# sdiehl/sonic

Measured on AMD Instinct MI355X. Metric: prove() proofs/sec, higher is better.
Workload: dtype u32 limbs (Fq 12x32, Fr 8x32 Montgomery); 1 GPU; prove(): rndCircuit n=2^18, Q=2, SRS d=2^21 (d=8n >= 7n, Protocol.hs:54); n=262144, Q=2, d=2097152, process_group=none (plain single-process run), legs=headline only (the other legs: --full)

## Files before the change

### include/sonic_hip.h

```cpp
#ifndef SONIC_HIP_H
#define SONIC_HIP_H
#include <stddef.h>
#include <stdint.h>

#if defined(__GNUC__)
#pragma GCC visibility push(default)
#endif
#ifdef __cplusplus
extern "C" {
#endif

enum {
  SONIC_OK = 0,
  SONIC_ERR_D_TOO_SMALL = 1,
  SONIC_ERR_SRS_INDEX = 2,
  SONIC_ERR_BAD_ENCODING = 3,
  SONIC_ERR_INEXACT_DIVISION = 4,
  SONIC_ERR_HIP = 5,
  SONIC_ERR_NO_DEVICE = 6,
  SONIC_ERR_INVALID_ARG = 7
};

#define SONIC_FR_BYTES 32
#define SONIC_G1_BYTES 96
// ... 47 lines not shown
int sonic_msm_g1_srs(const sonic_srs_t* srs, int basis, int64_t e0, const uint8_t* scalars, int64_t n,
                     uint8_t out_g1[96]);
int sonic_msm_g1_srs_dev(const sonic_srs_t* srs, int basis, int64_t e0, const void* d_scalars, int64_t n,
                         uint8_t out_g1[96]);
int sonic_msm_g1_srs_partial_dev(const sonic_srs_t* srs, int basis, int64_t e0, const void* d_scalars,
                                 int64_t n, uint8_t out_partial[192]);
int sonic_msm_g2(const uint8_t* points , const uint8_t* scalars , int64_t n, uint8_t out_g2[192]);
int sonic_msm_g2_srs(const sonic_srs_t* srs, int basis, int64_t e0, const uint8_t* scalars, int64_t n, uint8_t out_g2[192]);
int sonic_msm_g2_srs_dev(const sonic_srs_t* srs, int basis, int64_t e0, const void* d_scalars, int64_t n, uint8_t out_g2[192]);
int sonic_msm_g2_walk_max(void);
typedef struct sonic_msm_lane sonic_msm_lane_t;
int sonic_msm_lane_new(sonic_msm_lane_t** out);
int sonic_msm_lane_new_on(int device, sonic_msm_lane_t** out);
void sonic_msm_lane_free(sonic_msm_lane_t* lane);
int sonic_msm_submit(sonic_msm_lane_t* lane, const sonic_srs_t* srs, int basis, int64_t e0, const void* d_scalars, int64_t n);
int sonic_msm_collect(sonic_msm_lane_t* lane, uint8_t* out_g1, uint8_t* out_partial);
int sonic_msm_lane_new_on_stream(void* hip_stream, sonic_msm_lane_t** out);
int sonic_msm_submit_dev_v2(sonic_msm_lane_t* lane, const sonic_srs_t* srs, int basis, int64_t e0, const void* d_scalars, int64_t n,
                            void* d_partial_out, size_t out_bytes);
int sonic_msm_submit_dev(sonic_msm_lane_t* lane, const sonic_srs_t* srs, int basis, int64_t e0, const void* d_scalars, int64_t n,
                         void* d_partial_out);
int sonic_msm_exchange_layout(const sonic_srs_t* srs, int world, int64_t* n_buckets, int64_t* slice_len);
int sonic_msm_accumulate_dev(sonic_msm_lane_t* lane, const sonic_srs_t* srs, int basis, int64_t e0, const void* d_scalars, int64_t n,
                             void* d_buckets, int64_t capacity);
int sonic_msm_reduce_slices_dev_v2(sonic_msm_lane_t* lane, const sonic_srs_t* srs, const void* d_slices, int k, int64_t slice_len,
                                   int64_t bucket_base, void* d_partial_out, size_t out_bytes);
int sonic_msm_reduce_slices_dev(sonic_msm_lane_t* lane, const sonic_srs_t* srs, const void* d_slices, int k, int64_t slice_len,
                                int64_t bucket_base, void* d_partial_out);
int sonic_msm_lane_sync(sonic_msm_lane_t* lane);
int sonic_g1_sum_partials(const uint8_t* partials, int k, uint8_t out_g1[96]);
int sonic_g1_sum_dev_partials(const uint8_t* blobs, int k, uint8_t out_g1[96]);
int sonic_ntt_fr(uint8_t* data, int log2n, int inverse);
int sonic_poly_mul_fr(const uint8_t* a, int64_t na, const uint8_t* b, int64_t nb, uint8_t* out);
int sonic_poly_mul_fr_dev(const void* d_a, int64_t na, const void* d_b, int64_t nb, void* d_out);
int sonic_srs_point_bytes(void);
int sonic_msm_set_window(int c);
int sonic_msm_plan(const sonic_srs_t* srs, int64_t n, int* window_bits, int* windows, int* bucket_sets);

size_t sonic_proof_size(int64_t Q);
int sonic_prove(const sonic_srs_t* srs, int64_t n, int64_t Q, const uint8_t* wL, const uint8_t* wR,
                const uint8_t* wO, const uint8_t* cs, const uint8_t* aL, const uint8_t* aR,
                const uint8_t* aO, const uint8_t* transcript, uint8_t* out_proof);
int sonic_one_shot_trim(int device);
int sonic_prover_new(const sonic_srs_t* srs, int64_t n, int64_t Q, const uint8_t* wL, const uint8_t* wR,
                     const uint8_t* wO, const uint8_t* cs, sonic_prover_t** out);
int sonic_prover_new_csr(const sonic_srs_t* srs, int64_t n, int64_t Q, const int64_t* row_ptr, const int64_t* col, const uint8_t* val,
                         const uint8_t* cs, sonic_prover_t** out);
int sonic_prove_csr(const sonic_srs_t* srs, int64_t n, int64_t Q, const int64_t* row_ptr, const int64_t* col, const uint8_t* val,
                    const uint8_t* cs, const uint8_t* aL, const uint8_t* aR, const uint8_t* aO, const uint8_t* transcript,
                    uint8_t* out_proof);
int sonic_prover_set_assignment(sonic_prover_t* p, const uint8_t* aL, const uint8_t* aR, const uint8_t* aO);
int sonic_prover_prepare(sonic_prover_t* p);
int sonic_prover_prove(sonic_prover_t* p, const uint8_t* transcript, uint8_t* out_proof);
int sonic_prover_submit(sonic_prover_t* p, const uint8_t* transcript);
int sonic_prover_collect(sonic_prover_t* p, uint8_t* out_proof);
void sonic_prover_free(sonic_prover_t* p);

int sonic_prover_set_share(sonic_prover_t* p, int rank, int world);
size_t sonic_proof_share_size(int64_t Q);
int sonic_prover_prove_share(sonic_prover_t* p, const uint8_t* transcript, uint8_t* out_share);
int sonic_prover_collect_share(sonic_prover_t* p, uint8_t* out_share);
int sonic_proof_from_shares(int64_t Q, int world, const uint8_t* shares, const uint8_t* transcript, uint8_t* out_proof);
int sonic_prove_share_plan(int64_t n, int64_t Q, int prepared, int world, int rank, int64_t nb, int w, uint32_t* out_lo_hi, double* out_cost);

typedef struct sonic_statement {
  const uint8_t *wL, *wR, *wO, *cs;
// ... 190 lines not shown
```

### sonic_amd/_lib.py

```python
from __future__ import annotations

import ctypes as C
import os
import sys
import warnings

_HERE = os.path.dirname(os.path.abspath(__file__))
LIB_PATH = os.environ.get("SONIC_HIP_LIB") or os.path.join(_HERE, "csrc", "libsonic_hip.so")

ERR_NAMES = {
    1: "D_TOO_SMALL", 2: "SRS_INDEX_OUT_OF_RANGE", 3: "BAD_ENCODING", 4: "INEXACT_DIVISION",
    5: "HIP_ERROR", 6: "NO_DEVICE", 7: "INVALID_ARG",
}


class SonicError(RuntimeError):
    def __init__(self, code: int, message: str):
        super().__init__(f"{ERR_NAMES.get(code, code)}: {message}")
        self.code = code
        self.message = message


_lib = None

# ... 44 lines not shown
        "sonic_prove_batch": [vp, i32, i64, vp, vp, vp, vp, vp, vp],
        "sonic_prove_many": [vp, i32, i64, i64, vp, i64, vp, vp],
        "sonic_one_shot_trim": [i32],
        "sonic_msm_g1_srs_multi": [vp, i32, i32, i64, vp, i64, i32, vp],
        "sonic_msm_g1_srs_multi_dev": [vp, i32, i32, vp, vp, vp, i32, vp],
        "sonic_prover_device": [vp],
        "sonic_dev_alloc_on": [i32, C.c_size_t, C.POINTER(vp)],
        "sonic_srs_get_points": [vp, i32, i64, i64, vp],
        "sonic_srs_get_g2_points": [vp, i32, i64, i64, vp],
        "sonic_srs_save": [vp, cp, i32],
        "sonic_srs_has_g2": [vp],
        "sonic_srs_set_g2_points": [vp, vp, vp],
        "sonic_srs_load": [cp, C.POINTER(vp)],
        "sonic_commit_poly": [vp, i64, i64, vp, vp, vp],
        "sonic_open_poly": [vp, cp, i64, vp, vp, vp, vp],
        "sonic_msm_g1": [vp, vp, i64, vp],
        "sonic_msm_g1_srs": [vp, i32, i64, vp, i64, vp],
        "sonic_msm_g1_srs_dev": [vp, i32, i64, vp, i64, vp],
        "sonic_msm_g1_srs_partial_dev": [vp, i32, i64, vp, i64, vp],
        "sonic_g1_sum_partials": [vp, i32, vp],
        "sonic_g1_sum_dev_partials": [vp, i32, vp],
        "sonic_msm_lane_new": [C.POINTER(vp)],
        "sonic_msm_submit": [vp, vp, i32, i64, vp, i64],
        "sonic_msm_collect": [vp, vp, vp],
        "sonic_msm_lane_new_on_stream": [vp, C.POINTER(vp)],
        "sonic_msm_submit_dev_v2": [vp, vp, i32, i64, vp, i64, vp, C.c_size_t],
        "sonic_msm_exchange_layout": [vp, i32, C.POINTER(i64), C.POINTER(i64)],
        "sonic_msm_accumulate_dev": [vp, vp, i32, i64, vp, i64, vp, i64],
        "sonic_msm_reduce_slices_dev_v2": [vp, vp, vp, i32, i64, i64, vp, C.c_size_t],
        "sonic_msm_lane_sync": [vp],
        "sonic_ntt_fr": [vp, i32, i32],
        "sonic_poly_mul_fr": [vp, i64, vp, i64, vp],
        "sonic_poly_mul_fr_dev": [vp, i64, vp, i64, vp],
        "sonic_msm_set_window": [i32],
        "sonic_srs_point_bytes": [],
        "sonic_msm_plan": [vp, i64, C.POINTER(i32), C.POINTER(i32), C.POINTER(i32)],
        "sonic_prove": [vp, i64, i64] + [vp] * 9,
        "sonic_prover_new": [vp, i64, i64, vp, vp, vp, vp, C.POINTER(vp)],
        "sonic_prover_new_csr": [vp, i64, i64, vp, vp, vp, vp, C.POINTER(vp)],
        "sonic_prove_csr": [vp, i64, i64] + [vp] * 9,
        "sonic_fs_circuit_digest_csr": [i64, i64, vp, vp, vp, vp, vp],
        "sonic_verify_csr": [vp, i64, i64, vp, vp, vp, vp, vp, cp, cp, vp, C.POINTER(i32)],
        "sonic_verify_fs_csr": [vp, i64, i64, vp, vp, vp, vp, vp, C.POINTER(i32)],
        "sonic_prover_set_assignment": [vp, vp, vp, vp],
        "sonic_prover_prove": [vp, vp, vp],
        "sonic_prover_submit": [vp, vp],
        "sonic_prover_collect": [vp, vp],
        "sonic_prover_prepare": [vp],
        "sonic_prover_set_share": [vp, i32, i32],
        "sonic_prover_prove_share": [vp, vp, vp],
        "sonic_prover_collect_share": [vp, vp],
        "sonic_proof_from_shares": [i64, i32, vp, vp, vp],
        "sonic_prove_share_plan": [i64, i64, i32, i32, i32, i64, i32, vp, C.POINTER(C.c_double)],
        "sonic_fs_circuit_digest": [i64, i64, vp, vp, vp, vp, vp],
        "sonic_prover_prove_fs": [vp, cp, cp, vp, vp],
        "sonic_fs_srs_id": [vp, vp],
        "sonic_fs_challenges_v2": [i64, i64, i64, cp, cp, vp, vp],
        "sonic_verify_fs": [vp, i64, i64, vp, vp, vp, vp, vp, C.POINTER(i32)],
        "sonic_prover_hsc_prove": [vp, i64, vp, cp, cp, vp],
        "sonic_hsc_prove_poly": [vp, i64, vp, vp, vp, i64, vp, cp, cp, vp],
        "sonic_hsc_verify_poly": [vp, i64, vp, vp, vp, i64, vp, vp, C.POINTER(i32)],
        "sonic_hsc_verify": [vp, i64, i64, vp, vp, vp, i64, vp, vp, C.POINTER(i32)],
        "sonic_pc_v": [vp, i64, cp, cp, cp, cp, C.POINTER(i32)],
        "sonic_verify": [vp, i64, i64, vp, vp, vp, vp, vp, cp, cp, vp, C.POINTER(i32)],
        "sonic_verifier_new": [vp, i64, i64, vp, vp, vp, vp, C.POINTER(vp)],
        "sonic_verifier_new_csr": [vp, i64, i64, vp, vp, vp, vp, C.POINTER(vp)],
# ... 140 lines not shown
EXPORTED = [
    "sonic_abi_version", "sonic_device_count", "sonic_srs_new_on", "sonic_srs_from_points_on", "sonic_srs_replicate", "sonic_srs_device", "sonic_srs_pairing",
    "sonic_srs_load_on", "sonic_msm_lane_new_on", "sonic_msm_submit_dev_v2", "sonic_msm_reduce_slices_dev_v2", "sonic_fs_challenges_v2",
    "sonic_prove_shared", "sonic_prove_batch", "sonic_prove_many", "sonic_one_shot_trim", "sonic_msm_g1_srs_multi", "sonic_msm_g1_srs_multi_dev", "sonic_prover_device", "sonic_dev_alloc_on",
    "sonic_init", "sonic_last_error", "sonic_device_sync", "sonic_hip_versions", "sonic_srs_new", "sonic_srs_from_points",
    "sonic_srs_free", "sonic_srs_d", "sonic_srs_get_points", "sonic_srs_get_g2_points", "sonic_srs_set_g2_points", "sonic_srs_save", "sonic_srs_has_g2", "sonic_srs_load", "sonic_commit_poly", "sonic_open_poly",
    "sonic_msm_g1", "sonic_msm_g1_srs", "sonic_msm_g1_srs_dev", "sonic_msm_g1_srs_partial_dev",
    "sonic_g1_sum_partials", "sonic_g1_sum_dev_partials", "sonic_msm_lane_new", "sonic_msm_lane_free", "sonic_msm_submit", "sonic_msm_collect", "sonic_msm_lane_new_on_stream", "sonic_msm_submit_dev", "sonic_msm_exchange_layout",
    "sonic_msm_accumulate_dev", "sonic_msm_reduce_slices_dev", "sonic_msm_lane_sync", "sonic_ntt_fr", "sonic_poly_mul_fr", "sonic_poly_mul_fr_dev", "sonic_msm_set_window", "sonic_srs_point_bytes", "sonic_msm_plan",
    "sonic_proof_size", "sonic_prove", "sonic_prover_new", "sonic_prover_set_assignment",
    "sonic_prover_prove", "sonic_prover_submit", "sonic_prover_collect", "sonic_prover_prepare",
    "sonic_prover_set_share", "sonic_proof_share_size", "sonic_prover_prove_share", "sonic_prover_collect_share", "sonic_proof_from_shares", "sonic_prove_share_plan", "sonic_fs_circuit_digest", "sonic_fs_srs_id", "sonic_prover_prove_fs", "sonic_fs_challenges", "sonic_verify_fs", "sonic_prover_hsc_prove", "sonic_hsc_prove_poly", "sonic_hsc_verify_poly", "sonic_hsc_proof_size", "sonic_hsc_verify", "sonic_prover_free", "sonic_pc_v", "sonic_verify", "sonic_dev_alloc", "sonic_dev_free", "sonic_dev_upload",
    "sonic_dev_download", "sonic_profile_enable", "sonic_profile_reset", "sonic_profile_get",
    "sonic_profile_names",
    "sonic_prover_new_csr", "sonic_prove_csr", "sonic_fs_circuit_digest_csr", "sonic_verify_csr", "sonic_verify_fs_csr",
    "sonic_verifier_new", "sonic_verifier_new_csr", "sonic_verifier_free", "sonic_verifier_device", "sonic_verifier_verify_batch", "sonic_verifier_verify_fs_batch",
    "sonic_verifier_eval_s", "sonic_g1_validate", "sonic_verify_batch_randomizers",
    "sonic_g1_compress", "sonic_g1_decompress", "sonic_g2_compress", "sonic_g2_decompress", "sonic_proof_size_compressed", "sonic_proof_compress", "sonic_proof_decompress",
    "sonic_verifier_verify_batch_z", "sonic_verifier_verify_fs_batch_z", "sonic_srs_save_compressed",
    "sonic_prover_eval_constraints", "sonic_prover_set_constants", "sonic_prove_batch_statements", "sonic_fs_circuit_midstate", "sonic_fs_circuit_midstate_csr",
    "sonic_fs_circuit_digest_resume", "sonic_verifier_verify_batch_cs", "sonic_verifier_verify_fs_batch_cs", "sonic_verify_batch_digest_v2",
    "sonic_prover_witness_digest_v2", "sonic_prover_submit_fs", "sonic_prover_collect_fs", "sonic_prove_batch_fs",
    "sonic_prover_set_witness", "sonic_prover_eval_constraints_src", "sonic_prove_batch_src", "sonic_prove_batch_fs_src",
    "sonic_srs_for_circuit", "sonic_srs_load_for_circuit", "sonic_srs_load_for_circuit_on", "sonic_srs_windows", "sonic_srs_device_bytes",
    "sonic_prover_prove_core", "sonic_prover_submit_core", "sonic_prover_collect_core", "sonic_prover_prove_core_fs", "sonic_fs_core_challenges",
    "sonic_prove_batch_core_src", "sonic_prove_batch_core_fs_src", "sonic_verify_core", "sonic_verify_core_csr", "sonic_verify_core_fs", "sonic_verify_core_fs_csr",
    "sonic_verifier_verify_core_batch", "sonic_verifier_verify_core_fs_batch", "sonic_verify_core_batch_digest", "sonic_core_proof_compress", "sonic_core_proof_decompress",
    "sonic_fs_weights_digest", "sonic_fs_aggregate_challenges", "sonic_prover_aggregate_core", "sonic_verify_core_helped_digest",
    "sonic_verifier_verify_core_batch_helped", "sonic_verifier_verify_core_fs_batch_helped",
    "sonic_srs_check", "sonic_srs_update", "sonic_srs_verify_update",
    "sonic_msm_g2", "sonic_msm_g2_srs", "sonic_msm_g2_srs_dev", "sonic_msm_g2_walk_max",
    "sonic_g1_subgroup_check", "sonic_g2_subgroup_check",
    "sonic_pairing_check",
]


def last_error() -> str:
    buf = C.create_string_buffer(512)
    lib().sonic_last_error(buf, 512)
    return buf.value.decode(errors="replace")


def check(rc: int) -> None:
    if rc != 0:
        raise SonicError(rc, last_error())
```

### sonic_amd/csrc/poly.hip

```cpp
#include "internal.hpp"
#include "poly.hpp"
#include "csr.hpp"

namespace sonic {

#ifndef SONIC_SCALE_PER
#define SONIC_SCALE_PER 32
#endif
constexpr int SCALE_PER = SONIC_SCALE_PER;
static int scale_per(long n) {
  long per = n / (256L * 64L);
  if (per > SCALE_PER) per = SCALE_PER;
  if (per < 2) per = 2;
  return (int)per;
}

template <int MODE>
__global__ __launch_bounds__(256) void k_scale_powers(const Fr* __restrict__ in, Fr* __restrict__ out, long n, long e0,
                                                      const Fr* __restrict__ px, const Fr* __restrict__ pxinv, long lo_q, long nF, int PER) {
  const long base = (long)blockIdx.x * (256 * PER) + threadIdx.x;
  if (base >= n) return;
  const Fr x = *px, xinv = *pxinv;
  const long e = e0 + base;
  Fr p = e >= 0 ? fp_pow_u64(x, (uint64_t)e) : fp_pow_u64(xinv, (uint64_t)(-e));
// ... 59 lines not shown
  __shared__ Fr sh[256];
  __shared__ Fr carry_sh;
  if (threadIdx.x == 0) carry_sh = Fr::zero();
  __syncthreads();
  for (long base = 0; base < ntiles; base += 256) {
    long idx = base + threadIdx.x;
    Fr v = idx < ntiles ? tile_sums[idx] : Fr::zero();
    Fr incl = block_inclusive_scan_fr(v, sh);
    Fr carry = carry_sh;
    if (idx < ntiles) tile_sums[idx] = fp_add(fp_sub(incl, v), carry);
    __syncthreads();
    if (threadIdx.x == 255) carry_sh = fp_add(carry, incl);
    __syncthreads();
  }
}
__global__ __launch_bounds__(256) void k_prefix_apply(Fr* __restrict__ d, long n, const Fr* __restrict__ tile_sums) {
  const long i = (long)blockIdx.x * 256 + threadIdx.x;
  if (i >= n) return;
  const long tile = i >> 10;
  if (tile == 0) return;
  d[i] = fp_add(d[i], tile_sums[tile]);
}
void poly_prefix_sum_enqueue(hipStream_t st, Fr* d, long n, DevBuf& tmp) {
  if (n <= 0) return;
  const long ntiles = (n + 1023) / 1024;
  tmp.ensure(sizeof(Fr) * (ntiles + 1));
  LAUNCH(k_prefix_tiles, (int)ntiles, 256, 0, st, d, n, tmp.as<Fr>());
  if (ntiles > 1) {
    LAUNCH(k_prefix_top, 1, 256, 0, st, tmp.as<Fr>(), ntiles);
    LAUNCH(k_prefix_apply, ceil_div(n, 256), 256, 0, st, d, n, (const Fr*)tmp.as<Fr>());
  }
}

template <int MODE>
__global__ __launch_bounds__(256) void k_scale_powers_b(const OpenBatch b, long n, long e0, long lo_q, long nF, int PER, int tile_log) {
  const int y = blockIdx.y;
  const long base = (long)blockIdx.x * (256 * PER) + threadIdx.x;
  const Fr* __restrict__ in = MODE == 0 ? b.poly[y] : b.D[y];
  const Fr* __restrict__ tiles = b.tiles[y];
  Fr* __restrict__ out = MODE == 0 ? b.D[y] : b.q[y];
  Fr F;
  if (MODE == 2) {
    F = in[nF - 1];
    if (((nF - 1) >> tile_log) > 0) F = fp_add(F, tiles[(nF - 1) >> tile_log]);
    if (blockIdx.x == 0 && threadIdx.x == 0) *b.fz[y] = F;
  }
  if (base >= n) return;
  const Fr x = MODE == 0 ? b.zpair[y][0] : b.zpair[y][1], xinv = MODE == 0 ? b.zpair[y][1] : b.zpair[y][0];
  const long e = e0 + base;
  Fr p = e >= 0 ? fp_pow_u64(x, (uint64_t)e) : fp_pow_u64(xinv, (uint64_t)(-e));
  const Fr step = fp_pow_u64(x, 256);
#pragma unroll 1
  for (int k = 0; k < PER; k++) {
    const long i = base + (long)k * 256;
    if (i >= n) break;
    Fr v;
    if (MODE == 0) v = fp_mul(in[i], p);
    else {
      Fr P = in[i];
      if ((i >> tile_log) > 0) P = fp_add(P, tiles[i >> tile_log]);
      v = fp_mul((lo_q + i >= 0) ? fp_sub(F, P) : fp_neg(P), p);
    }
    out[i] = v;
    p = fp_mul(p, step);
  }
}
template <int EPT>
__global__ __launch_bounds__(256) void k_prefix_tiles_b(const OpenBatch b, long n) {
  __shared__ Fr sh[256];
  Fr* __restrict__ d = b.D[blockIdx.y];
  const long base = (long)blockIdx.x * (256 * EPT) + threadIdx.x * EPT;
  Fr s = Fr::zero();
  for (int k = 0; k < EPT; k++) if (base + k < n) s = fp_add(s, d[base + k]);
  Fr incl = block_inclusive_scan_fr(s, sh);
  Fr run = fp_sub(incl, s);
  for (int k = 0; k < EPT; k++) if (base + k < n) { run = fp_add(run, d[base + k]); d[base + k] = run; }
  if (threadIdx.x == 255) b.tiles[blockIdx.y][blockIdx.x] = incl;
}
__global__ __launch_bounds__(256) void k_prefix_top_b(const OpenBatch b, long ntiles) {
  __shared__ Fr sh[256];
  __shared__ Fr carry_sh;
  Fr* __restrict__ tile_sums = b.tiles[blockIdx.x];
  if (threadIdx.x == 0) carry_sh = Fr::zero();
  __syncthreads();
  for (long base = 0; base < ntiles; base += 256) {
    long idx = base + threadIdx.x;
    Fr v = idx < ntiles ? tile_sums[idx] : Fr::zero();
    Fr incl = block_inclusive_scan_fr(v, sh);
    Fr carry = carry_sh;
    if (idx < ntiles) tile_sums[idx] = fp_add(fp_sub(incl, v), carry);
    __syncthreads();
    if (threadIdx.x == 255) carry_sh = fp_add(carry, incl);
    __syncthreads();
  }
}
__global__ void k_last_prefix_b(const OpenBatch b, long len, int tile_log) {
  const int y = blockIdx.x;
  Fr F = b.D[y][len - 1];
  if (((len - 1) >> tile_log) > 0) F = fp_add(F, b.tiles[y][(len - 1) >> tile_log]);
  *b.fz[y] = F;
}
void open_batch_enqueue(hipStream_t st, const OpenBatch& b, long lo, long len, bool quotient) {
  if (b.k <= 0 || len <= 0) return;
  const unsigned k = (unsigned)b.k;
  const int tile_log = len >= 65536 ? 12 : 10;
  const int per = scale_per(len);
  LAUNCH(k_scale_powers_b<0>, dim3((unsigned)ceil_div(len, 256L * per), k), 256, 0, st, b, len, lo, 0L, 0L, per, tile_log);
  const long ntiles = (len + (1L << tile_log) - 1) >> tile_log;
  if (tile_log == 12) LAUNCH(k_prefix_tiles_b<16>, dim3((unsigned)ntiles, k), 256, 0, st, b, len);
  else LAUNCH(k_prefix_tiles_b<4>, dim3((unsigned)ntiles, k), 256, 0, st, b, len);
  if (ntiles > 1) LAUNCH(k_prefix_top_b, k, 256, 0, st, b, ntiles);
  if (!quotient) { LAUNCH(k_last_prefix_b, k, 1, 0, st, b, len, tile_log); return; }
  const long qn = len > 1 ? len - 1 : 1;
  const int per2 = scale_per(qn);
  LAUNCH(k_scale_powers_b<2>, dim3((unsigned)ceil_div(qn, 256L * per2), k), 256, 0, st, b, len - 1 > 0 ? len - 1 : 0, 1 + lo, lo, len, per2, tile_log);
}

__global__ __launch_bounds__(256) void k_build_r1(const Fr* __restrict__ aL, const Fr* __restrict__ aR, const Fr* __restrict__ aO,
                                                  const Fr* __restrict__ cns, long n, Fr* __restrict__ r1) {
  const long len = 3 * n + 5;
  for (long i = (long)blockIdx.x * 256 + threadIdx.x; i < len; i += (long)gridDim.x * 256) {
    const long e = i - (2 * n + 4);
    Fr v = Fr::zero();
    if (e > 0) v = aL[e - 1];
    else if (e < 0 && e >= -n) v = aR[-e - 1];
    else if (e < -n && e >= -2 * n) v = aO[-e - n - 1];
    else if (e < -2 * n) v = cns[-e - 2 * n - 1];
    r1[i] = v;
  }
}
void build_r1_enqueue(hipStream_t st, const Fr* aL, const Fr* aR, const Fr* aO, const Fr* cns, long n, Fr* r1) {
  LAUNCH(k_build_r1, elementwise_grid(3 * n + 5), 256, 0, st, aL, aR, aO, cns, n, r1);
}

__global__ __launch_bounds__(256) void k_s_of_y(const Fr* __restrict__ wL, const Fr* __restrict__ wR, const Fr* __restrict__ wO,
                                                const Fr* __restrict__ ypow, long n, long Q, Fr* __restrict__ s) {
  for (long i = (long)blockIdx.x * 256 + threadIdx.x + 1; i <= n + 1; i += (long)gridDim.x * 256) {
    if (i > n) { s[n] = Fr::zero(); break; }
    Fr u = Fr::zero(), v = Fr::zero(), w = Fr::zero();
    for (long q = 0; q < Q; q++) {
      const Fr yq = ypow[2 * n + 1 + q];
      u = fp_add(u, fp_mul(wL[q * n + i - 1], yq));
      v = fp_add(v, fp_mul(wR[q * n + i - 1], yq));
      w = fp_add(w, fp_mul(wO[q * n + i - 1], yq));
    }
    w = fp_sub(fp_sub(w, ypow[n + i]), ypow[n - i]);
    s[n - i] = u;
    s[n + i] = v;
// ... 311 lines not shown
```

### sonic_amd/csrc/poly.hpp

```cpp
#pragma once
#include "common.hpp"
#include "field.hpp"
#include "g1.hpp"

namespace sonic {

void build_r1_enqueue(hipStream_t st, const Fr* aL, const Fr* aR, const Fr* aO, const Fr* cns, long n, Fr* r1);
void s_of_y_enqueue(hipStream_t st, const Fr* wL, const Fr* wR, const Fr* wO, const Fr* ypow, long n, long Q, Fr* s);
void weight_row_poly_enqueue(hipStream_t st, const Fr* wL, const Fr* wR, const Fr* wO, long n, long q, Fr* s);
void s_diag_part_enqueue(hipStream_t st, const Fr* ypow, long n, long Q, Fr* diag, Fr* yq);
void s_of_u_enqueue(hipStream_t st, const Fr* wL, const Fr* wR, const Fr* wO, const Fr* upow, long n, long Q, Fr* s, DevBuf& tmp);
void s_of_y_csc_enqueue(hipStream_t st, const int32_t* col_ptr, const int32_t* row, const Fr* val, const Fr* ypow, long n, long Q, Fr* s);
void s_of_u_csr_enqueue(hipStream_t st, const int32_t* row_ptr, const int32_t* col, const Fr* val, const int32_t* chunk_row, const int32_t* chunk_begin,
                        long nchunks, const int32_t* row_chunk, const Fr* upow, long n, long Q, Fr* s, Fr* partial);
void csr_row_terms_enqueue(hipStream_t st, const int32_t* col, const Fr* val, const int32_t seg[6], long n, PointArray A, G1Affine* pts, Fr* scal);
void add_into_enqueue(hipStream_t st, Fr* dst, const Fr* src, long n);
void t_operands_enqueue(hipStream_t st, const Fr* r1, long r_len, long r_lo, const Fr* sy, long s_off, long s_len, const Fr* ypair, Fr* fa, Fr* fb, long M);
void sub_k_of_y_enqueue(hipStream_t st, Fr* slot, const Fr* cs, const Fr* ypow_nq, long Q, int* flags, int flag_bit);
void flag_nonzero_enqueue(hipStream_t st, const Fr* a, long n, int* flags, int bit);
constexpr int RUN_TILE = 256;
void run_tiles_enqueue(hipStream_t st, const Fr* poly, long len, Fr* masked, Fr* val, uint32_t* uniform);
void run_terms_enqueue(hipStream_t st, const Fr* val, const uint32_t* uniform, long ntiles, PointArray ps, long ps_first, Fr* scal, G1Affine* pts);
void fr_with_inverse_enqueue(hipStream_t st, const Fr* in, int k, Fr* out);
void fr_mul_scalar_enqueue(hipStream_t st, const Fr* a, const Fr* b, Fr* out);
void scale_terms_enqueue(hipStream_t st, const int64_t* e, const Fr* c, long nt, const Fr* pair, Fr* out);
void sparse_to_dense_enqueue(hipStream_t st, const int64_t* exps, const Fr* coeffs, long nt, long lo, Fr* dense);

constexpr int OPEN_BATCH_MAX = 16;
struct OpenBatch {
  int k;
  const Fr* poly[OPEN_BATCH_MAX];
  Fr* D[OPEN_BATCH_MAX];
  Fr* q[OPEN_BATCH_MAX];
  Fr* tiles[OPEN_BATCH_MAX];
  const Fr* zpair[OPEN_BATCH_MAX];
  Fr* fz[OPEN_BATCH_MAX];
};
void open_batch_enqueue(hipStream_t st, const OpenBatch& b, long lo, long len, bool quotient = true);

}
```

### sonic_amd/csrc/poly_api.hip

```cpp
#include "prover.hpp"

extern "C" {

struct BivTerms {
  long nt = 0, lo = 0, len = 0;
  DevBuf keep, other, coeff;
};
static int biv_upload(hipStream_t st, int64_t nt, const int64_t* keep, const int64_t* other, const uint8_t* coeffs, BivTerms& out, int* d_flags) {
  out.nt = nt;
  long lo = 0, hi = 0;
  for (int64_t i = 0; i < nt; i++) { lo = std::min<long>(lo, keep[i]); hi = std::max<long>(hi, keep[i]); }
  out.lo = lo; out.len = hi - lo + 1;
  std::vector<int64_t> order(nt), k(nt), o(nt);
  std::iota(order.begin(), order.end(), 0);
  std::stable_sort(order.begin(), order.end(), [&](int64_t a, int64_t b) { return keep[a] < keep[b]; });
  std::vector<uint8_t> c(32 * (size_t)(nt ? nt : 1));
  for (int64_t i = 0; i < nt; i++) { k[i] = keep[order[i]]; o[i] = other[order[i]]; memcpy(&c[32 * (size_t)i], coeffs + 32 * order[i], 32); }
  out.keep.alloc(8 * (size_t)(nt ? nt : 1)); out.other.alloc(8 * (size_t)(nt ? nt : 1)); out.coeff.alloc(32 * (size_t)(nt ? nt : 1));
  if (nt) {
    HIP_OK(hipMemcpyAsync(out.keep.p, k.data(), 8 * (size_t)nt, hipMemcpyHostToDevice, st));
    HIP_OK(hipMemcpyAsync(out.other.p, o.data(), 8 * (size_t)nt, hipMemcpyHostToDevice, st));
    HIP_OK(hipMemcpyAsync(out.coeff.p, c.data(), 32 * (size_t)nt, hipMemcpyHostToDevice, st));
    fr_to_mont_enqueue(st, out.coeff.as<Fr>(), nt, d_flags);
  }
// ... 205 lines not shown
}

int sonic_poly_mul_fr(const uint8_t* a, int64_t na, const uint8_t* b, int64_t nb, uint8_t* out) {
  API_BEGIN
  if (!a || !b || !out || na < 1 || nb < 1) return SONIC_ERR_INVALID_ARG;
  std::lock_guard<std::mutex> g(call_mutex());
  hipStream_t st = default_stream();
  const long rl = na + nb - 1;
  int lg = 0;
  while ((1L << lg) < rl) lg++;
  const long M = 1L << lg;
  DevBuf fa(sizeof(Fr) * M), fb(sizeof(Fr) * M), flags(4);
  HIP_OK(hipMemsetAsync(flags.p, 0, 4, st));
  HIP_OK(hipMemsetAsync(fa.p, 0, sizeof(Fr) * M, st));
  HIP_OK(hipMemsetAsync(fb.p, 0, sizeof(Fr) * M, st));
  HIP_OK(hipMemcpyAsync(fa.p, a, 32 * na, hipMemcpyHostToDevice, st));
  HIP_OK(hipMemcpyAsync(fb.p, b, 32 * nb, hipMemcpyHostToDevice, st));
  fr_to_mont_enqueue(st, fa.as<Fr>(), na, flags.as<int>());
  fr_to_mont_enqueue(st, fb.as<Fr>(), nb, flags.as<int>());
  if (lg > 0) {
    shared_ntt().ensure(st, lg);
    ntt_forward_enqueue(st, shared_ntt(), fa.as<Fr>(), lg);
    ntt_forward_enqueue(st, shared_ntt(), fb.as<Fr>(), lg);
  }
  if (lg > 0) ntt_inverse_of_product_enqueue(st, shared_ntt(), fa.as<Fr>(), fb.as<Fr>(), lg);
  else fr_pointwise_mul_enqueue(st, fa.as<Fr>(), fb.as<Fr>(), M);
  fr_from_mont_enqueue(st, fa.as<Fr>(), rl);
  int fl = read_flags(st, flags);
  if (fl) return flags_to_status(fl, "sonic_poly_mul_fr");
  HIP_OK(hipMemcpy(out, fa.p, 32 * rl, hipMemcpyDeviceToHost));
  API_END
}

int sonic_poly_mul_fr_dev(const void* d_a, int64_t na, const void* d_b, int64_t nb, void* d_out) {
  API_BEGIN
  if (!d_a || !d_b || !d_out || na < 1 || nb < 1) return SONIC_ERR_INVALID_ARG;
  std::lock_guard<std::mutex> g(call_mutex());
  hipStream_t st = default_stream();
  const long rl = na + nb - 1;
  int lg = 0;
  while ((1L << lg) < rl) lg++;
  const long M = 1L << lg;
  DeviceCtx& dctx = current_ctx();
  DevBuf *fa = &dctx.mul_a, *fb = &dctx.mul_b, *flags = &dctx.mul_flags;
  fa->ensure(sizeof(Fr) * M); fb->ensure(sizeof(Fr) * M); flags->ensure(4);
  HIP_OK(hipMemsetAsync(flags->p, 0, 4, st));
  HIP_OK(hipMemsetAsync(fa->p, 0, sizeof(Fr) * M, st));
  HIP_OK(hipMemsetAsync(fb->p, 0, sizeof(Fr) * M, st));
  HIP_OK(hipMemcpyAsync(fa->p, d_a, 32 * na, hipMemcpyDeviceToDevice, st));
  HIP_OK(hipMemcpyAsync(fb->p, d_b, 32 * nb, hipMemcpyDeviceToDevice, st));
  fr_to_mont_enqueue(st, fa->as<Fr>(), na, flags->as<int>());
  fr_to_mont_enqueue(st, fb->as<Fr>(), nb, flags->as<int>());
  if (lg > 0) {
    shared_ntt().ensure(st, lg);
    ntt_forward_enqueue(st, shared_ntt(), fa->as<Fr>(), lg);
    ntt_forward_enqueue(st, shared_ntt(), fb->as<Fr>(), lg);
  }
  if (lg > 0) ntt_inverse_of_product_enqueue(st, shared_ntt(), fa->as<Fr>(), fb->as<Fr>(), lg);
  else fr_pointwise_mul_enqueue(st, fa->as<Fr>(), fb->as<Fr>(), M);
  fr_from_mont_enqueue(st, fa->as<Fr>(), rl);
  HIP_OK(hipMemcpyAsync(d_out, fa->p, 32 * rl, hipMemcpyDeviceToDevice, st));
  int fl = read_flags(st, *flags);
  if (fl) return flags_to_status(fl, "sonic_poly_mul_fr_dev");
  API_END
}

// ... 2 lines not shown
```

### sonic_amd/csrc/prove.hip

```cpp
#include "prover.hpp"
#include "witness_tree.hpp"

namespace sonic {

constexpr long PROVE_TWO_LEVEL_MAX_TERMS = 1L << 21;
constexpr long POOL_MAX_TERMS = 1L << 21;
static bool prove_two_level(const MsmPlan& pl, int k, bool last, long nmax) {
  if (last || k <= 1 || pl.NB < (1 << 18)) return false;
  const char* e = getenv("SONIC_PROVE_TWO_LEVEL");
  if (e && (e[0] == '0' || e[0] == '1') && !e[1]) return e[0] == '1';
  return nmax <= PROVE_TWO_LEVEL_MAX_TERMS;
}
static int prove_segment(const MsmPlan& pl, int k, bool last, bool two_level) {
  const bool big = pl.NB >= (1 << 18);
  if (last) return big ? 16 : 4;
  if (k <= 1) return big ? 8 : 4;
  if (!big) return 16;
  const char* e = getenv("SONIC_PROVE_SEGMENT");
  const int v = e ? atoi(e) : 0;
  return v >= 8 && v <= 1024 ? v : (two_level ? 32 : 64);
}

MsmJob commit_job(hipStream_t st, const sonic_srs* srs, const Fr* poly, long lo, long len, long maxm, MsmSlot* slot, int* d_flags) {
  const long d = srs->d, shift = d - maxm;
// ... 40 lines not shown

static MsmJob quotient_job(hipStream_t st, const sonic_srs* srs, const Fr* q, long lo, long len, MsmSlot* slot, int* d_flags) {
  const long d = srs->d, qn = len - 1;
  long i0 = -d - lo, i1 = d - lo + 1;
  if (i0 < 0) i0 = 0;
  if (i1 > qn) i1 = qn;
  if (i1 < i0) i1 = i0;
  const PointArray points = srs_job_points("openPoly", srs, 0, lo + i0, i1 - i0);
  flag_nonzero_enqueue(st, q, i0, d_flags, FLAG_SRS_INDEX);
  flag_nonzero_enqueue(st, q + i1, qn - i1, d_flags, FLAG_SRS_INDEX);
  return MsmJob{points, q + i0, i1 - i0, slot};
}

MsmJob open_job(hipStream_t st, const sonic_srs* srs, Scratch& sc, const Fr* poly, long lo, long len,
                       const Fr* zpair, Fr* d_fz, MsmSlot* slot, int* d_flags) {
  sc.reserve(len);
  eval_prefix_enqueue(st, sc, poly, lo, len, zpair, d_fz ? d_fz : sc.fz_discard.as<Fr>());
  poly_quotient_enqueue(st, sc.D.as<Fr>(), sc.q.as<Fr>(), len, lo, zpair, zpair + 1);
  return quotient_job(st, srs, sc.q.as<Fr>(), lo, len, slot, d_flags);
}

MsmJob open_job_at_zero(hipStream_t st, const sonic_srs* srs, const Fr* poly, long len, Fr* d_fz, MsmSlot* slot, int* d_flags) {
  const long d = srs->d;
  HIP_OK(hipMemcpyAsync(d_fz, poly, sizeof(Fr), hipMemcpyDeviceToDevice, st));
  const long qn = len - 1;
  long i1 = d + 1;
  if (i1 > qn) i1 = qn;
  flag_nonzero_enqueue(st, poly + 1 + i1, qn - i1, d_flags, FLAG_SRS_INDEX);
  return MsmJob{srs_job_points("openPoly", srs, 0, 0, i1), poly + 1, i1, slot};
}

struct PendingOpen { const Fr* poly; long lo, len; const Fr* zp; Fr* fz; MsmSlot* slot; long slot_index; Scratch* sc; };
static void open_batch_set(OpenBatch& b, int i, Scratch& sc, const Fr* poly, long len, const Fr* zp, Fr* fz) {
  sc.reserve(len);
  sc.scan.ensure(sizeof(Fr) * (len / 1024 + 2));
  b.poly[i] = poly; b.D[i] = sc.D.as<Fr>(); b.q[i] = sc.q.as<Fr>(); b.tiles[i] = sc.scan.as<Fr>();
  b.zpair[i] = zp; b.fz[i] = fz ? fz : sc.fz_discard.as<Fr>();
}
static void open_jobs_batched(hipStream_t st, const sonic_srs* srs, const PendingOpen* ops, int k, int* d_flags, MsmJob* jobs_out) {
  for (int at = 0; at < k;) {
    int e = at;
    OpenBatch b;
    memset(&b, 0, sizeof b);
    while (e < k && e - at < OPEN_BATCH_MAX && ops[e].lo == ops[at].lo && ops[e].len == ops[at].len) {
      open_batch_set(b, e - at, *ops[e].sc, ops[e].poly, ops[e].len, ops[e].zp, ops[e].fz);
      e++;
    }
    b.k = e - at;
    const long lo = ops[at].lo, len = ops[at].len;
    open_batch_enqueue(st, b, lo, len);
    for (int i = at; i < e; i++) jobs_out[i] = quotient_job(st, srs, ops[i].sc->q.as<Fr>(), lo, len, ops[i].slot, d_flags);
    at = e;
  }
}

bool bytes_are_zero(const uint8_t* p, size_t n) { for (size_t i = 0; i < n; i++) if (p[i]) return false; return true; }

}

int upload_fr_mont(hipStream_t st, DevBuf& dst, const uint8_t* src, long count, int* d_flags) {
  dst.ensure(sizeof(Fr) * (count > 0 ? count : 1));
  if (count > 0) {
    HIP_OK(hipMemcpyAsync(dst.p, src, 32 * count, hipMemcpyHostToDevice, st));
    fr_to_mont_enqueue(st, dst.as<Fr>(), count, d_flags);
  }
  return 0;
}

int flags_to_status(int f, const char* who) {
// ... 1475 lines not shown
```

Measured before the change: 31.18 proofs/s.

## Replace power-scaled prefix-scan opening with two-sided Horner sweep scan

Batched polynomial opening (evaluation at z plus quotient by (X - z)) used to scale coefficients by powers of z, prefix-scan them, and rescale. It now runs a chunked Horner-style linear-recurrence scan in both directions from degree zero: per-thread chunks, a block scan weighted by powers of z, a carry pass across tiles, and a final quotient pass. This removes the per-element pow computations and the D scratch buffer, at the cost of a sequential chunk loop per thread and a single-block carry kernel. A new host API for dense batch opening is also added.

```diff
diff --git a/include/sonic_hip.h b/include/sonic_hip.h
--- a/include/sonic_hip.h
+++ b/include/sonic_hip.h
@@ -103,6 +103,8 @@
 int sonic_g1_sum_dev_partials(const uint8_t* blobs, int k, uint8_t out_g1[96]);
 int sonic_ntt_fr(uint8_t* data, int log2n, int inverse);
 int sonic_poly_mul_fr(const uint8_t* a, int64_t na, const uint8_t* b, int64_t nb, uint8_t* out);
+int sonic_open_batch_dense(int k, const uint8_t* const* polys, int64_t lo, int64_t len, const uint8_t* zs, int quotient, int chunk,
+                           uint8_t* out_fz, uint8_t* const* out_q);
 int sonic_poly_mul_fr_dev(const void* d_a, int64_t na, const void* d_b, int64_t nb, void* d_out);
 int sonic_srs_point_bytes(void);
 int sonic_msm_set_window(int c);
diff --git a/sonic_amd/_lib.py b/sonic_amd/_lib.py
--- a/sonic_amd/_lib.py
+++ b/sonic_amd/_lib.py
@@ -100,6 +100,7 @@
         "sonic_ntt_fr": [vp, i32, i32],
         "sonic_poly_mul_fr": [vp, i64, vp, i64, vp],
         "sonic_poly_mul_fr_dev": [vp, i64, vp, i64, vp],
+        "sonic_open_batch_dense": [i32, vp, i64, i64, vp, i32, i32, vp, vp],
         "sonic_msm_set_window": [i32],
         "sonic_srs_point_bytes": [],
         "sonic_msm_plan": [vp, i64, C.POINTER(i32), C.POINTER(i32), C.POINTER(i32)],
@@ -306,6 +307,7 @@
     "sonic_msm_g2", "sonic_msm_g2_srs", "sonic_msm_g2_srs_dev", "sonic_msm_g2_walk_max",
     "sonic_g1_subgroup_check", "sonic_g2_subgroup_check",
     "sonic_pairing_check",
+    "sonic_open_batch_dense",
 ]
 
 
diff --git a/sonic_amd/csrc/poly.hip b/sonic_amd/csrc/poly.hip
--- a/sonic_amd/csrc/poly.hip
+++ b/sonic_amd/csrc/poly.hip
@@ -115,88 +115,137 @@
   }
 }
 
-template <int MODE>
-__global__ __launch_bounds__(256) void k_scale_powers_b(const OpenBatch b, long n, long e0, long lo_q, long nF, int PER, int tile_log) {
-  const int y = blockIdx.y;
-  const long base = (long)blockIdx.x * (256 * PER) + threadIdx.x;
-  const Fr* __restrict__ in = MODE == 0 ? b.poly[y] : b.D[y];
-  const Fr* __restrict__ tiles = b.tiles[y];
-  Fr* __restrict__ out = MODE == 0 ? b.D[y] : b.q[y];
-  Fr F;
-  if (MODE == 2) {
-    F = in[nF - 1];
-    if (((nF - 1) >> tile_log) > 0) F = fp_add(F, tiles[(nF - 1) >> tile_log]);
-    if (blockIdx.x == 0 && threadIdx.x == 0) *b.fz[y] = F;
-  }
-  if (base >= n) return;
-  const Fr x = MODE == 0 ? b.zpair[y][0] : b.zpair[y][1], xinv = MODE == 0 ? b.zpair[y][1] : b.zpair[y][0];
-  const long e = e0 + base;
-  Fr p = e >= 0 ? fp_pow_u64(x, (uint64_t)e) : fp_pow_u64(xinv, (uint64_t)(-e));
-  const Fr step = fp_pow_u64(x, 256);
+struct SweepShape {
+  long len, i0;
+  int L;
+  long M[2], nb[2], pad[2];
+};
+static SweepShape sweep_shape(long lo, long len, int chunk) {
+  SweepShape s;
+  s.len = len; s.i0 = -lo; s.L = chunk ? chunk : open_sweep_chunk(len);
+  const long tile = (long)SWEEP_BLOCK * s.L;
+  s.M[0] = s.i0; s.M[1] = len - 1 - s.i0;
+  for (int r = 0; r < 2; r++) { s.nb[r] = ceil_div(s.M[r], tile); s.pad[r] = s.nb[r] * tile - s.M[r]; }
+  return s;
+}
+template <bool UP>
+__device__ __forceinline__ Fr sweep_step(const Fr& x, const Fr& a, const Fr& m) {
+  return UP ? fp_mul(fp_sub(x, a), m) : fp_add(a, fp_mul(x, m));
+}
+template <bool UP, bool STORE>
+__device__ __forceinline__ Fr sweep_chunk(const Fr* __restrict__ f, Fr* __restrict__ q, long t0, int L, long top, Fr x, const Fr& m) {
 #pragma unroll 1
-  for (int k = 0; k < PER; k++) {
-    const long i = base + (long)k * 256;
-    if (i >= n) break;
-    Fr v;
-    if (MODE == 0) v = fp_mul(in[i], p);
-    else {
-      Fr P = in[i];
-      if ((i >> tile_log) > 0) P = fp_add(P, tiles[i >> tile_log]);
-      v = fp_mul((lo_q + i >= 0) ? fp_sub(F, P) : fp_neg(P), p);
+  for (int g = 0; g < L; g += 4) {
+    Fr a[4];
+#pragma unroll
+    for (int j = 0; j < 4; j++) {
+      const long t = t0 + g + j;
+      a[j] = (g + j < L && t >= 0) ? f[UP ? t : top - t] : Fr::zero();
     }
-    out[i] = v;
-    p = fp_mul(p, step);
-  }
-}
-template <int EPT>
-__global__ __launch_bounds__(256) void k_prefix_tiles_b(const OpenBatch b, long n) {
-  __shared__ Fr sh[256];
-  Fr* __restrict__ d = b.D[blockIdx.y];
-  const long base = (long)blockIdx.x * (256 * EPT) + threadIdx.x * EPT;
-  Fr s = Fr::zero();
-  for (int k = 0; k < EPT; k++) if (base + k < n) s = fp_add(s, d[base + k]);
-  Fr incl = block_inclusive_scan_fr(s, sh);
-  Fr run = fp_sub(incl, s);
-  for (int k = 0; k < EPT; k++) if (base + k < n) { run = fp_add(run, d[base + k]); d[base + k] = run; }
-  if (threadIdx.x == 255) b.tiles[blockIdx.y][blockIdx.x] = incl;
-}
-__global__ __launch_bounds__(256) void k_prefix_top_b(const OpenBatch b, long ntiles) {
-  __shared__ Fr sh[256];
-  __shared__ Fr carry_sh;
-  Fr* __restrict__ tile_sums = b.tiles[blockIdx.x];
-  if (threadIdx.x == 0) carry_sh = Fr::zero();
-  __syncthreads();
-  for (long base = 0; base < ntiles; base += 256) {
-    long idx = base + threadIdx.x;
-    Fr v = idx < ntiles ? tile_sums[idx] : Fr::zero();
-    Fr incl = block_inclusive_scan_fr(v, sh);
-    Fr carry = carry_sh;
-    if (idx < ntiles) tile_sums[idx] = fp_add(fp_sub(incl, v), carry);
-    __syncthreads();
-    if (threadIdx.x == 255) carry_sh = fp_add(carry, incl);
-    __syncthreads();
-  }
-}
-__global__ void k_last_prefix_b(const OpenBatch b, long len, int tile_log) {
-  const int y = blockIdx.x;
-  Fr F = b.D[y][len - 1];
-  if (((len - 1) >> tile_log) > 0) F = fp_add(F, b.tiles[y][(len - 1) >> tile_log]);
-  *b.fz[y] = F;
-}
-void open_batch_enqueue(hipStream_t st, const OpenBatch& b, long lo, long len, bool quotient) {
+#pragma unroll
+    for (int j = 0; j < 4; j++) {
+      const long t = t0 + g + j;
+      if (g + j < L && t >= 0) {
+        x = sweep_step<UP>(x, a[j], m);
+        if (STORE) q[UP ? t : top - 1 - t] = x;
+      }
+    }
+  }
+  return x;
+}
+__global__ __launch_bounds__(SWEEP_BLOCK) void k_sweep_chunks_b(const OpenBatch b, const SweepShape s) {
+  __shared__ Fr sh[SWEEP_BLOCK];
+  __shared__ Fr mu[9];
+  const int y = blockIdx.y, t = threadIdx.x;
+  const int r = (long)blockIdx.x >= s.nb[0];
+  const long tile = (long)blockIdx.x - (r ? s.nb[0] : 0), NB = s.nb[0] + s.nb[1];
+  const Fr m = b.zpair[y][r ? 0 : 1];
+  Fr* __restrict__ base = b.tiles[y];
+  if (t < 64) {
+    Fr p = fp_pow_u64(m, (uint64_t)s.L);
+    for (int k = 0; k < 9; k++) {
+      if (t == 0) mu[k] = p;
+      if (k < 8) p = fp_mul(p, p);
+    }
+  }
+  const long t0 = (tile * SWEEP_BLOCK + t) * s.L - s.pad[r];
+  sh[t] = r == 0 ? sweep_chunk<true, false>(b.poly[y], nullptr, t0, s.L, 0, Fr::zero(), m)
+                 : sweep_chunk<false, false>(b.poly[y], nullptr, t0, s.L, s.len - 1, Fr::zero(), m);
+  __syncthreads();
+  for (int k = 0, o = 1; o < SWEEP_BLOCK; o <<= 1, k++) {
+    const Fr x = t >= o ? sh[t - o] : Fr::zero();
+    __syncthreads();
+    sh[t] = fp_add(sh[t], fp_mul(x, mu[k]));
+    __syncthreads();
+  }
+  base[(long)blockIdx.x * SWEEP_BLOCK + t] = t > 0 ? sh[t - 1] : Fr::zero();
+  if (t == SWEEP_BLOCK - 1) base[NB * SWEEP_BLOCK + blockIdx.x] = sh[t];
+  if (tile == 0 && s.nb[r] > 1) {
+    Fr p = Fr::one();
+    for (int k = 0; k < 8; k++) if ((t >> k) & 1) p = fp_mul(p, mu[k]);
+    Fr* __restrict__ pw = base + NB * (SWEEP_BLOCK + 1) + r * (SWEEP_BLOCK + 1);
+    pw[t] = p;
+    if (t == 0) pw[SWEEP_BLOCK] = mu[8];
+  }
+}
+__global__ __launch_bounds__(2 * SWEEP_BLOCK) void k_sweep_carries_b(const OpenBatch b, const SweepShape s) {
+  __shared__ Fr sh[2][SWEEP_BLOCK];
+  __shared__ Fr fin[2];
+  const int y = blockIdx.x, r = threadIdx.x / SWEEP_BLOCK, u = threadIdx.x % SWEEP_BLOCK;
+  const long NB = s.nb[0] + s.nb[1], nt = s.nb[r], most = s.nb[0] > s.nb[1] ? s.nb[0] : s.nb[1];
+  Fr* __restrict__ base = b.tiles[y];
+  Fr* __restrict__ tt = base + NB * SWEEP_BLOCK + (r ? s.nb[0] : 0);
+  Fr last = Fr::zero();
+  if (most <= 1) {
+    if (nt == 1) last = tt[0];
+  } else {
+    const Fr muT = nt > 1 ? base[NB * (SWEEP_BLOCK + 1) + r * (SWEEP_BLOCK + 1) + SWEEP_BLOCK] : Fr::zero();
+    Fr carry = Fr::zero();
+    for (long bs = 0; bs < most; bs += SWEEP_BLOCK) {
+      const long idx = bs + u;
+      Fr v = idx < nt ? tt[idx] : Fr::zero();
+      if (u == 0) v = fp_add(v, fp_mul(carry, muT));
+      sh[r][u] = v;
+      __syncthreads();
+      Fr mu = muT;
+      for (int o = 1; o < SWEEP_BLOCK; o <<= 1) {
+        const Fr x = u >= o ? sh[r][u - o] : Fr::zero();
+        __syncthreads();
+        sh[r][u] = fp_add(sh[r][u], fp_mul(x, mu));
+        __syncthreads();
+        mu = fp_mul(mu, mu);
+      }
+      if (idx < nt) tt[idx] = u > 0 ? sh[r][u - 1] : carry;
+      if (nt - 1 >= bs && nt - 1 < bs + SWEEP_BLOCK) last = sh[r][nt - 1 - bs];
+      carry = sh[r][SWEEP_BLOCK - 1];
+      __syncthreads();
+    }
+  }
+  if (u == 0) fin[r] = last;
+  __syncthreads();
+  if (threadIdx.x == 0) *b.fz[y] = fp_sub(fp_add(b.poly[y][s.i0], fp_mul(b.zpair[y][0], fin[1])), fin[0]);
+}
+__global__ __launch_bounds__(SWEEP_BLOCK) void k_sweep_quotient_b(const OpenBatch b, const SweepShape s) {
+  const int y = blockIdx.y, t = threadIdx.x;
+  const int r = (long)blockIdx.x >= s.nb[0];
+  const long tile = (long)blockIdx.x - (r ? s.nb[0] : 0), NB = s.nb[0] + s.nb[1];
+  const long t0 = (tile * SWEEP_BLOCK + t) * s.L - s.pad[r];
+  if (t0 + s.L <= 0) return;
+  const Fr m = b.zpair[y][r ? 0 : 1];
+  const Fr* __restrict__ base = b.tiles[y];
+  Fr x = base[(long)blockIdx.x * SWEEP_BLOCK + t];
+  if (tile > 0) x = fp_add(x, fp_mul(base[NB * (SWEEP_BLOCK + 1) + r * (SWEEP_BLOCK + 1) + t], base[NB * SWEEP_BLOCK + blockIdx.x]));
+  if (r == 0) sweep_chunk<true, true>(b.poly[y], b.q[y], t0, s.L, 0, x, m);
+  else sweep_chunk<false, true>(b.poly[y], b.q[y], t0, s.L, s.len - 1, x, m);
+}
+void open_batch_enqueue(hipStream_t st, const OpenBatch& b, long lo, long len, bool quotient, int chunk) {
   if (b.k <= 0 || len <= 0) return;
   const unsigned k = (unsigned)b.k;
-  const int tile_log = len >= 65536 ? 12 : 10;
-  const int per = scale_per(len);
-  LAUNCH(k_scale_powers_b<0>, dim3((unsigned)ceil_div(len, 256L * per), k), 256, 0, st, b, len, lo, 0L, 0L, per, tile_log);
-  const long ntiles = (len + (1L << tile_log) - 1) >> tile_log;
-  if (tile_log == 12) LAUNCH(k_prefix_tiles_b<16>, dim3((unsigned)ntiles, k), 256, 0, st, b, len);
-  else LAUNCH(k_prefix_tiles_b<4>, dim3((unsigned)ntiles, k), 256, 0, st, b, len);
-  if (ntiles > 1) LAUNCH(k_prefix_top_b, k, 256, 0, st, b, ntiles);
-  if (!quotient) { LAUNCH(k_last_prefix_b, k, 1, 0, st, b, len, tile_log); return; }
-  const long qn = len > 1 ? len - 1 : 1;
-  const int per2 = scale_per(qn);
-  LAUNCH(k_scale_powers_b<2>, dim3((unsigned)ceil_div(qn, 256L * per2), k), 256, 0, st, b, len - 1 > 0 ? len - 1 : 0, 1 + lo, lo, len, per2, tile_log);
+  const SweepShape s = sweep_shape(lo, len, chunk);
+  const unsigned NB = (unsigned)(s.nb[0] + s.nb[1]);
+  if (NB) LAUNCH(k_sweep_chunks_b, dim3(NB, k), SWEEP_BLOCK, 0, st, b, s);
+  LAUNCH(k_sweep_carries_b, k, 2 * SWEEP_BLOCK, 0, st, b, s);
+  if (quotient && NB) LAUNCH(k_sweep_quotient_b, dim3(NB, k), SWEEP_BLOCK, 0, st, b, s);
 }
 
 __global__ __launch_bounds__(256) void k_build_r1(const Fr* __restrict__ aL, const Fr* __restrict__ aR, const Fr* __restrict__ aO,
diff --git a/sonic_amd/csrc/poly.hpp b/sonic_amd/csrc/poly.hpp
--- a/sonic_amd/csrc/poly.hpp
+++ b/sonic_amd/csrc/poly.hpp
@@ -27,15 +27,24 @@
 void sparse_to_dense_enqueue(hipStream_t st, const int64_t* exps, const Fr* coeffs, long nt, long lo, Fr* dense);
 
 constexpr int OPEN_BATCH_MAX = 16;
+constexpr int SWEEP_BLOCK = 256;
+constexpr int SWEEP_CHUNK_MAX = 16;
+inline int open_sweep_chunk(long len) {
+  const long L = len / ((long)SWEEP_BLOCK * 64);
+  return (int)(L > SWEEP_CHUNK_MAX ? SWEEP_CHUNK_MAX : (L < 2 ? 2 : L));
+}
+inline long open_sweep_entries(long len, int chunk = 0) {
+  const long tile = (long)SWEEP_BLOCK * (chunk ? chunk : open_sweep_chunk(len));
+  return (len / tile + 2) * (SWEEP_BLOCK + 1) + 2 * (SWEEP_BLOCK + 1);
+}
 struct OpenBatch {
   int k;
   const Fr* poly[OPEN_BATCH_MAX];
-  Fr* D[OPEN_BATCH_MAX];
   Fr* q[OPEN_BATCH_MAX];
   Fr* tiles[OPEN_BATCH_MAX];
   const Fr* zpair[OPEN_BATCH_MAX];
   Fr* fz[OPEN_BATCH_MAX];
 };
-void open_batch_enqueue(hipStream_t st, const OpenBatch& b, long lo, long len, bool quotient = true);
+void open_batch_enqueue(hipStream_t st, const OpenBatch& b, long lo, long len, bool quotient = true, int chunk = 0);
 
 }
diff --git a/sonic_amd/csrc/poly_api.hip b/sonic_amd/csrc/poly_api.hip
--- a/sonic_amd/csrc/poly_api.hip
+++ b/sonic_amd/csrc/poly_api.hip
@@ -261,6 +261,52 @@
   API_END
 }
 
+int sonic_open_batch_dense(int k, const uint8_t* const* polys, int64_t lo, int64_t len, const uint8_t* zs, int quotient, int chunk,
+                           uint8_t* out_fz, uint8_t* const* out_q) {
+  API_BEGIN
+  if (k < 1 || k > OPEN_BATCH_MAX || (chunk != 0 && (chunk < 2 || chunk > SWEEP_CHUNK_MAX)) || !polys || !zs || !out_fz || len < 1 || lo > 0 || lo + len - 1 < 0 || (quotient && len > 1 && !out_q))
+    return SONIC_ERR_INVALID_ARG;
+  for (int i = 0; i < k; i++) {
+    if (!polys[i] || (quotient && len > 1 && !out_q[i])) return SONIC_ERR_INVALID_ARG;
+    if (bytes_are_zero(zs + 32 * i, 32)) { set_error("sonic_open_batch_dense: z_%d = 0 (the chain divides by z)", i); return SONIC_ERR_INEXACT_DIVISION; }
+  }
+  std::lock_guard<std::mutex> g(call_mutex());
+  hipStream_t st = default_stream();
+  DevBuf flags(4), zin(sizeof(Fr) * k), zpair(2 * sizeof(Fr) * k), fz(sizeof(Fr) * k);
+  std::vector<DevBuf> f((size_t)k), q((size_t)k), tiles((size_t)k);
+  HIP_OK(hipMemsetAsync(flags.p, 0, 4, st));
+  HIP_OK(hipMemcpyAsync(zin.p, zs, 32 * (size_t)k, hipMemcpyHostToDevice, st));
+  fr_to_mont_enqueue(st, zin.as<Fr>(), k, flags.as<int>());
+  fr_with_inverse_enqueue(st, zin.as<Fr>(), k, zpair.as<Fr>());
+  OpenBatch b;
+  memset(&b, 0, sizeof b);
+  b.k = k;
+  for (int i = 0; i < k; i++) {
+    int same = -1;
+    for (int j = 0; j < i && same < 0; j++) if (polys[j] == polys[i]) same = j;
+    if (same < 0) {
+      f[i].alloc(sizeof(Fr) * len);
+      HIP_OK(hipMemcpyAsync(f[i].p, polys[i], 32 * (size_t)len, hipMemcpyHostToDevice, st));
+      fr_to_mont_enqueue(st, f[i].as<Fr>(), len, flags.as<int>());
+      b.poly[i] = f[i].as<Fr>();
+    } else {
+      b.poly[i] = b.poly[same];
+    }
+    q[i].alloc(sizeof(Fr) * (len + 1));
+    tiles[i].alloc(sizeof(Fr) * open_sweep_entries(len, chunk));
+    b.q[i] = q[i].as<Fr>(); b.tiles[i] = tiles[i].as<Fr>();
+    b.zpair[i] = zpair.as<Fr>() + 2 * i; b.fz[i] = fz.as<Fr>() + i;
+  }
+  open_batch_enqueue(st, b, lo, len, quotient != 0, chunk);
+  fr_from_mont_enqueue(st, fz.as<Fr>(), k);
+  if (quotient) for (int i = 0; i < k; i++) fr_from_mont_enqueue(st, q[i].as<Fr>(), len - 1);
+  int fl = read_flags(st, flags);
+  if (fl) return flags_to_status(fl, "sonic_open_batch_dense");
+  HIP_OK(hipMemcpy(out_fz, fz.p, 32 * (size_t)k, hipMemcpyDeviceToHost));
+  if (quotient && len > 1) for (int i = 0; i < k; i++) HIP_OK(hipMemcpy(out_q[i], q[i].p, 32 * (size_t)(len - 1), hipMemcpyDeviceToHost));
+  API_END
+}
+
 int sonic_poly_mul_fr_dev(const void* d_a, int64_t na, const void* d_b, int64_t nb, void* d_out) {
   API_BEGIN
   if (!d_a || !d_b || !d_out || na < 1 || nb < 1) return SONIC_ERR_INVALID_ARG;
diff --git a/sonic_amd/csrc/prove.hip b/sonic_amd/csrc/prove.hip
--- a/sonic_amd/csrc/prove.hip
+++ b/sonic_amd/csrc/prove.hip
@@ -96,9 +96,10 @@
 
 struct PendingOpen { const Fr* poly; long lo, len; const Fr* zp; Fr* fz; MsmSlot* slot; long slot_index; Scratch* sc; };
 static void open_batch_set(OpenBatch& b, int i, Scratch& sc, const Fr* poly, long len, const Fr* zp, Fr* fz) {
-  sc.reserve(len);
-  sc.scan.ensure(sizeof(Fr) * (len / 1024 + 2));
-  b.poly[i] = poly; b.D[i] = sc.D.as<Fr>(); b.q[i] = sc.q.as<Fr>(); b.tiles[i] = sc.scan.as<Fr>();
+  sc.q.ensure(sizeof(Fr) * (len + 1));
+  sc.fz_discard.ensure(sizeof(Fr));
+  sc.scan.ensure(sizeof(Fr) * open_sweep_entries(len));
+  b.poly[i] = poly; b.q[i] = sc.q.as<Fr>(); b.tiles[i] = sc.scan.as<Fr>();
   b.zpair[i] = zp; b.fz[i] = fz ? fz : sc.fz_discard.as<Fr>();
 }
 static void open_jobs_batched(hipStream_t st, const sonic_srs* srs, const PendingOpen* ops, int k, int* d_flags, MsmJob* jobs_out) {
```

After: 31.67 proofs/s (median of 6 runs). 1.02x the previous value.
